# zhouxian/act3d-chained-diffuser

Measured on AMD Instinct MI355X. Metric: train samples/sec (Act3D keypose fwd+bwd+AdamW step), higher is better.
Workload: dtype fp16 / bf16 MFMA on two-part operands (x = hi + lo; fp32 accumulate) in attention; fp32-accurate linears (f32 MFMA; bf16x3 MFMA from 4096 rows); bf16 frozen backbone + FPN; 1 GPU; Act3D keypose training step, 18-PerAct-task shapes: 4 cameras 256x256, 3 ghost-point levels, 1000 ghost points (333/level), E=60, frozen synthetic CLIP-RN50-shaped backbone + trainable FPN included in the step; per_gpu_batch_keyframes=64, global_batch=64, parallelism=dp1, hipgraph=True, backbone_prefetch=True

## Files before the change

### act3d-chained-diffuser_amd/build.py

```python
import os
import shutil
import subprocess
import sys
from concurrent.futures import ThreadPoolExecutor

PKG_DIR = os.path.dirname(os.path.abspath(__file__))
CSRC = os.path.join(PKG_DIR, "csrc")
OBJ_DIR = os.path.join(CSRC, "obj")
_OUT = os.path.basename(os.environ.get("A3D_LIB_OUT", "libact3d_hip.so"))
LIB_PATH = os.path.join(PKG_DIR, _OUT)
if _OUT != "libact3d_hip.so":
    OBJ_DIR = os.path.join(CSRC, "obj_" + _OUT[len("libact3d_hip_"):-3])
INCLUDE = os.path.join(os.path.dirname(PKG_DIR), "include")
SOURCES = ["api.hip", "linear.hip", "linear_split.hip", "rope.hip", "ctx_proj.hip", "attention.hip", "attention_bwd.hip", "attention16.hip", "attention8.hip", "scene.hip", "heads.hip", "optim.hip", "diffusion.hip", "traj_rank.hip", "traj_clearance.hip", "traj_guide.hip", "vision.hip", "dropout.hip", "denoise.hip", "single_query.hip", "single_query_wave.hip", "query_stream.hip", "data.hip", "conv1x1.hip", "conv1x1_deep.hip", "bn_gram.hip", "conv3x3.hip", "fpn_sparse.hip", "stem.hip"]
FLAGS = ["--offload-arch=gfx950", "-O3", "-std=c++17", "-fPIC", "-Wno-unused-result"]
_ATTN_FLAGS = ["-fno-honor-nans", "-mno-amdgpu-ieee"]
EXTRA_FLAGS = {"attention.hip": _ATTN_FLAGS, "attention_bwd.hip": _ATTN_FLAGS, "attention16.hip": _ATTN_FLAGS,
               "attention8.hip": _ATTN_FLAGS, "traj_clearance.hip": ["-Wall", "-Wextra"],
               "traj_guide.hip": ["-Wall", "-Wextra"], "optim.hip": ["-Wall", "-Wextra"]}


ENV_FLAGS = os.environ.get("A3D_HIPCC_FLAGS", "").split()


def _hipcc():
    for cand in (shutil.which("hipcc"), "/opt/rocm/bin/hipcc"):
        if cand and os.path.exists(cand):
            return cand
    raise RuntimeError("hipcc not found: libact3d_hip.so cannot be built on this machine")


def _newer(src, dst):
    return (not os.path.exists(dst)) or os.path.getmtime(src) > os.path.getmtime(dst)


def build(force=False, verbose=False):
    hipcc = _hipcc()
    os.makedirs(OBJ_DIR, exist_ok=True)
    deps = [os.path.join(CSRC, "a3d_common.h"), os.path.join(CSRC, "attn_ring.h"), os.path.join(CSRC, "traj_points.h"),
            os.path.join(INCLUDE, "act3d_hip.h"),
            os.path.abspath(__file__)]
    srcs = [s for s in SOURCES if os.path.exists(os.path.join(CSRC, s))]
    jobs = []
    for s in srcs:
        src = os.path.join(CSRC, s)
        obj = os.path.join(OBJ_DIR, s.replace(".hip", ".o"))
        if force or _newer(src, obj) or any(_newer(d, obj) for d in deps):
            jobs.append((src, obj))

    def compile_one(job):
        src, obj = job
        cmd = [hipcc] + FLAGS + EXTRA_FLAGS.get(os.path.basename(src), []) + ENV_FLAGS + ["-c", src, "-o", obj]
        r = subprocess.run(cmd, capture_output=True, text=True)
        if r.returncode != 0:
            raise RuntimeError("hipcc failed for %s:\n%s" % (src, r.stderr[-4000:]))
        if verbose:
            print("compiled", os.path.basename(src), file=sys.stderr)
        return obj

    if jobs:
        with ThreadPoolExecutor(max_workers=min(8, len(jobs))) as ex:
            list(ex.map(compile_one, jobs))
    objs = [os.path.join(OBJ_DIR, s.replace(".hip", ".o")) for s in srcs]
    if force or jobs or not os.path.exists(LIB_PATH):
        cmd = [hipcc, "--offload-arch=gfx950", "-shared", "-fPIC", "-o", LIB_PATH] + objs
        r = subprocess.run(cmd, capture_output=True, text=True)
        if r.returncode != 0:
            raise RuntimeError("link failed:\n%s" % r.stderr[-4000:])
    return LIB_PATH


if __name__ == "__main__":
    print(build(force="--force" in sys.argv, verbose=True))
```

### act3d-chained-diffuser_amd/lib.py

```python
import ctypes as C
import os

import torch

_PKG_DIR = os.path.dirname(os.path.abspath(__file__))
LIB_PATH = os.path.join(_PKG_DIR, os.path.basename(os.environ.get("A3D_LIB", "libact3d_hip.so")))

_p = C.c_void_p
_i = C.c_int
_f = C.c_float
_d = C.c_double
_z = C.c_size_t
_u64 = C.c_ulonglong



def _struct(name, fields):
    return type(name, (C.Structure,), {"_fields_": [(f, t) for f, t in fields]})


DnHeadParams = _struct("DnHeadParams", [(n, _p) for n in ("enc_w0", "enc_b0", "enc_w1", "enc_b1", "sem", "lang_kv")] +
                       [("S_lang", _i)] + [(n, _p) for n in ("q_w", "q_b", "out_w", "out_b", "ln_g", "ln_b")])
DnCrossParams = _struct("DnCrossParams", [(n, _p) for n in ("sem", "mod", "q_w", "q_b", "freq", "Kf", "Vt")])
DnRestParams = _struct("DnRestParams", [(n, _p) for n in (
# ... 58 lines not shown
    "a3d_traj_clearance_ws_floats": (_z, [_i] * 5),
    "a3d_traj_clearance": (_i, [_p, _p, _p, _p, _i, _i, _f, _i, _i, _p, _p, _p] + [_i] * 5 + [_p]),
    "a3d_traj_guide_ws_floats": (_z, [_i] * 5),
    "a3d_traj_guide": (_i, [_p, _i, _p, _p, _p, _p, _p, _i, _i, _f, _i, _i, _f, _f, _p, _p] + [_i] * 4 + [_p]),
    "a3d_traj_errors": (_i, [_p, _p, _p, _i, _i, _i, _p]),
    "a3d_keypose_errors": (_i, [_p, _p, _p, _p, _i, _p, _i, _i, _i, _p]),
    "a3d_sym_quat_loss": (_i, [_p, _p, _i, _f, _p, _p, _i, _p]),
    "a3d_sq_fwd_ws_floats": (_z, [_i, _i, _i, _i]),
    "a3d_sq_attn_fwd": (_i, [_p, _p, _p, _i, _p, _p, _i, _p, _p, _p, _p, _p, _p, _p, _i, _i, _i, _i, _i, _p]),
    "a3d_sq_bwd_ws_floats": (_z, [_i, _i, _i, _i]),
    "a3d_sq_attn_bwd": (_i, [_p, _p, _p, _i, _p, _p, _i, _p, _p, _p, _p, _p, _p, _p, _p, _p, _i, _p, _p, _i, _p, _i, _i, _i, _i,
                             _i, _p]),
    "a3d_sq_attn_bwd_acc": (_i, [_p, _p, _p, _i, _p, _p, _i, _p, _p, _p, _p, _p, _p, _p, _p, _p, _i, _p, _p, _i, _p, _i, _i, _i, _i,
                                 _i, _i, _p]),
    "a3d_qs_pre_fwd": (_i, [_p, _p, _p, _p, _p, _f, _p, _i, _i, _i, _p]),
    "a3d_qs_pre_bwd": (_i, [_p, _i, _p, _p, _f, _p, _p, _p, _p, _p, _i, _i, _i, _p]),
    "a3d_qs_save_floats": (_z, [_i, _i]),
    "a3d_qs_post_fwd": (_i, [_p, _p, _p, _p, _p, _i, _i, _i, _p]),
    "a3d_qs_post_bwd": (_i, [_p, _p, _p, _p, _p, _p, _p, _p, _p, _i, _i, _i, _p]),
    "a3d_sq_wgrad_reduce": (_i, [_p, _i, _p, _i, _p, _i, _p]),
    "a3d_dn_head": (_i, [_p, _i, _p, _p, _i, _i, _i, _i, _p]),
    "a3d_dn_cross_ws_floats": (_z, [_i, _i, _i]),
    "a3d_dn_cross": (_i, [_p, _p, _i, _p, _p, _i, _i, _i, _i, _i, _i, _i, _p]),
    "a3d_dn_rest": (_i, [_p, _p, _i, _p, _p, _p, _i, _i, _i, _i, _i, _p]),
    "a3d_dn_tail": (_i, [_p, _p, _p, _i, _p, _p, _i, _i, _i, _i, _p]),
    "a3d_dn_tail_sched": (_i, [_p, _p, _p, _i, _p, _p, _i, _i, _i, _i, _i, _p]),
    "a3d_dn_persist_splits": (_i, [_i, _i]),
    "a3d_dn_persist_sync_ints": (_z, [_i, _i, _i, _i]),
    "a3d_dn_persist_kvx_floats": (_z, [_i, _i, _i]),
    "a3d_dn_persist_prof": (_i, [_p, _i, _i, _i, _i, _p]),
    "a3d_dn_persist_xbuf_floats": (_z, [_i, _i]),
    "a3d_dn_persist": (_i, [_p, _i, _i, _i, _p, _p, _p, _p, _p, _p, _p, _p] + [_i] * 10 + [_p]),
    "a3d_dn_persist_sched": (_i, [_p, _i, _i, _i, _p, _p, _p, _p, _p, _p, _p, _p] + [_i] * 12 + [_p]),
    "a3d_dn_persist_group_of": (_i, [_i, _i, _i, _i, _p]),
    "a3d_dn_persist_group": (_i, [_p, _i, _i, _i, _p, _p, _p, _p, _p, _p, _p, _p] + [_i] * 13 + [_p]),
    "a3d_rope_rows_f32": (_i, [_p, _i, _p, _p, _f, _p, _i, _i, _i, _i, _i, _p]),
    "a3d_dropout": (_i, [_p, _p, _z, _p, C.c_uint, _f, _p]),
    "a3d_dropout_mask": (_i, [_p, _z, _p, C.c_uint, C.c_uint, C.c_uint, _f, _p]),
    "a3d_linear_fwd_drop": (_i, [_p, _i, _p, _i, _p, _p, _i, _p, _i, _i, _i, _i, _i, _i, _p, C.c_uint, _f, _p]),
    "a3d_add_layernorm_bwd_drop": (_i, [_p] * 10 + [_i, _i, _p, C.c_uint, _f, _p]),
    "a3d_attn_fwd_dropout": (_i, [_p, _p, _p, _p, _p, _p, _p, _i, _i, _i, _i, _i, _i, _i, _p, C.c_uint, _f, _p]),
    "a3d_attn_bwd_bf16_dropout": (_i, [_p] * 15 + [_i] * 7 + [_p, C.c_uint, _f, _p]),
    "a3d_pcd_downsample": (_i, [_p, _p, _i, _i, _i, _i, _i, _p]),
    "a3d_knn_topk_ws_bytes": (_z, [_i, _i]),
    "a3d_knn_topk": (_i, [_p, _p, _p, _p, _p, _i, _i, _i, _p]),
    "a3d_traj_nn_topk": (_i, [_p, _i, _p, _p, _p, _p, _i, _i, _i, _p]),
    "a3d_build_context": (_i, [_p, _p, _p, _p, _i, _i, _i, _i, _i, _p]),
    "a3d_build_context_bwd": (_i, [_p, _p, _p, _p, _i, _i, _i, _i, _i, _i, _p]),
    "a3d_build_context_bf16": (_i, [_p, _i, _p, _p, _p, _p, _i, _i, _i, _i, _i, _p]),
    "a3d_colsum_rows_ws_floats": (_z, [_i, _i, _i]),
    "a3d_colsum_rows": (_i, [_p, _i, _i, _i, _i, _i, _p, _i, _p, _p]),
    "a3d_build_context_bwd_bf16": (_i, [_p, _p, _p, _i, _p, _i, _i, _i, _i, _i, _i, _p]),
    "a3d_mask_logits_fwd": (_i, [_p, _p, _p, _i, _i, _i, _p]),
    "a3d_mask_logits_bwd": (_i, [_p, _p, _p, _p, _p, _i, _i, _i, _i, _p]),
    "a3d_argmax_gather": (_i, [_p, _p, _p, _p, _i, _i, _p]),
    "a3d_soft_ce_loss": (_i, [_p, _p, _p, _p, _p, _p, _i, _i, _f, _f, _f, _p]),
    "a3d_elem_loss": (_i, [_p, _p, _i, _i, _f, _p, _p, _p]),
    "a3d_scale_by_scalar": (_i, [_p, _p, _p, _z, _p]),
    "a3d_quat_sigmoid_fwd": (_i, [_p, _p, _p, _i, _p]),
    "a3d_quat_sigmoid_bwd": (_i, [_p, _p, _p, _p, _i, _p]),
    "a3d_ortho6d_sigmoid_fwd": (_i, [_p, _p, _p, _i, _p]),
    "a3d_ortho6d_sigmoid_bwd": (_i, [_p, _p, _p, _p, _i, _p]),
    "a3d_select_row_fwd": (_i, [_p, _p, _p, _i, _i, _i, _p]),
    "a3d_select_row_bwd": (_i, [_p, _p, _p, _i, _i, _i, _p]),
    "a3d_sample_ghost_points": (_i, [_p, _p, _p, _f, _p, _i, _i, _i, _i, _p]),
    "a3d_rng_advance": (_i, [_p, _u64, _p]),
    "a3d_philox4x32_10_host": (None, [_p, _p, _p]),
    "a3d_sincos_host": (None, [_p, _p, _p, _z]),
    "a3d_adamw_step": (_i, [_p, _p, _p, _p, _p, _p, _p, _i, _z, _z, _f, _f, _f, _f, _f, _f, _f, _p]),
    "a3d_adamw_ema_step": (_i, [_p] * 9 + [_i, _z, _z] + [_f] * 9 + [_p]),
    "a3d_adamw_clip_step": (_i, [_p] * 11 + [_i, _z, _z] + [_f] * 10 + [_p]),
    "a3d_adamw_sched_step": (_i, [_p] * 12 + [_i, _z, _z, _i] + [_d] * 3 + [_f] * 9 + [_p]),
    "a3d_swap_f32": (_i, [_p, _p, _z, _p]),
    "a3d_dbg_mfma_bf16": (_i, [_p, _p, _p, _p]),
    "a3d_dbg_mfma_f32": (_i, [_p, _p, _p, _p]),
    "a3d_dbg_cvt_pk_bf16": (_i, [_p, _p, _i, _p]),
    "a3d_bn_nslab": (_i, [_z, _i]),
    "a3d_bn_grid_cap": (_i, [_i]),
    "a3d_conv1x1_streams": (_i, [_i, _i]),
    "a3d_conv1x1_nslab": (_i, [_z, _i, _i]),
    "a3d_conv1x1_bn_fwd": (_i, [_p, _p, _p, _p, _i, _p, _p, _z, _i, _i, _p]),
    "a3d_conv1x1_topdown_serves": (_i, [_i, _i]),
    "a3d_conv1x1_topdown_fwd": (_i, [_p, _p, _p, _i, _p, _p, _z, _i, _i, _i, _i, _p]),
    "a3d_conv1x1_bn_residual_serves": (_i, [_i, _i]),
    "a3d_conv1x1_bn_residual_fwd": (_i, [_p, _p, _p, _p, _i, _p, _p, _p, _p, _p, _i, _i, _p, _z, _i, _i, _p]),
    "a3d_bn_gram_nslab": (_i, [_z, _i]),
    "a3d_bn_gram": (_i, [_p, _p, _p, _i, _p, _p, _z, _i, _i, _p]),
    "a3d_bn_gram_stats": (_i, [_p, _p, _i, _p, _i, _i, _p, _p, _p]),
    "a3d_conv3x3_serves": (_i, [_i, _i, _i, _i]),
    "a3d_conv1x1_deep_mode": (_i, [_i]),
    "a3d_stem_conv_nslab": (_i, [_z, _i, _i]),
    "a3d_stem_conv_bn_fwd": (_i, [_p, _p, _p, _p, _p, _p, _z, _i, _i, _p]),
    "a3d_conv3x3_nslab": (_i, [_z, _i, _i, _i, _i]),
    "a3d_conv3x3_bn_fwd": (_i, [_p, _p, _p, _p, _i, _p, _p, _z, _i, _i, _i, _i, _p]),
    "a3d_bn_stats": (_i, [_p, _p, _z, _i, _i, _p]),
    "a3d_bn_finalize": (_i, [_p, _i, _z, _i, _f, _f, _p, _p, _p, _p, _p, _p, _i, _p]),
    "a3d_bn_apply": (_i, [_p, _p, _p, _p, _p, _p, _p, _z, _i, _i, _p]),
    "a3d_bn_apply_pool2": (_i, [_p, _p, _p, _p, _p, _p, _i, _i, _i, _i, _i, _p]),
    "a3d_rgb_normalize_nhwc_bf16": (_i, [_p, _p, _p, _p, _z, _i, _i, _p]),
    "a3d_upsample2_add_fwd": (_i, [_p, _p, _p, _i, _p, _i, _i, _i, _i, _p]),
    "a3d_upsample2_add_bwd_ws_floats": (_z, [_i, _i, _i, _i]),
    "a3d_upsample2_add_bwd": (_i, [_p, _p, _p, _i, _p, _i, _i, _i, _i, _p]),
    "a3d_ddpm_add_noise": (_i, [_p, _p, _p, _p, _p, _p, _i, _i, _i, _i, _p]),
    "a3d_ddpm_step": (_i, [_p, _p, _p, _p, _p, _p, _p, _p, _i, _i, _i, _i, _p]),
    "a3d_ddpm_step_sched": (_i, [_p, _p, _p, _p, _p, _p, _p, _p, _i, _i, _i, _i, _i, _p]),
    "a3d_adaln_fwd": (_i, [_p, _p, _p, _i, _i, _i, _p]),
    "a3d_adaln_bwd": (_i, [_p, _p, _p, _p, _p, _i, _i, _i, _p]),
    "a3d_sinusoidal_emb": (_i, [_p, _p, _i, _i, _p]),
    "a3d_silu_fwd": (_i, [_p, _p, _z, _p]),
    "a3d_silu_bwd": (_i, [_p, _p, _p, _z, _p]),
    "a3d_add_rows": (_i, [_p, _p, _p, _i, _i, _i, _p]),
    "a3d_add_rows_bwd": (_i, [_p, _p, _i, _i, _i, _p]),
    "a3d_resize_crop": (_i, [_p, _p, _p, _i, _i, _i, _i, _f, _f, _p]),
    "a3d_traj_update": (_i, [_p, _p, _p, _i, _i, _i, _p]),
}

ADAMW_CLIP_WS_DOUBLES = 256
LR_DECAY_KINDS = {"constant": 0, "linear": 1, "cosine": 2}

_lib = None


def load():
    global _lib
    if _lib is not None:
        return _lib
    if not os.path.exists(LIB_PATH):
        raise RuntimeError(
            "libact3d_hip.so is missing (%s). Build it with `python -c 'import __graft_entry__ as g; g.build()'` "
            "(needs hipcc); there is no CPU fallback." % LIB_PATH)
    lib = C.CDLL(LIB_PATH)
    for name, (res, args) in SIGNATURES.items():
        try:
            fn = getattr(lib, name)
        except AttributeError as e:
            raise RuntimeError("libact3d_hip.so does not export %s (stale build?)" % name) from e
        fn.restype = res
        fn.argtypes = args
    _lib = lib
    return lib


def exported_symbols():
    return list(SIGNATURES.keys())


def last_error():
    s = load().a3d_last_error_string()
    return s.decode() if s else ""


def check(rc, what=""):
    if rc != 0:
        raise RuntimeError("libact3d_hip %s failed with code %d: %s" % (what, rc, last_error()))


def ptr(t):
    if t is None:
        return None
    assert t.is_contiguous(), "libact3d_hip needs contiguous tensors"
    return t.data_ptr()


def stream():
    return torch.cuda.current_stream().cuda_stream

# ... 14 lines not shown
```

### act3d-chained-diffuser_amd/nn.py

```python
import collections
import math
import os

import torch
import torch.nn as nn
import torch.nn.functional as F

from . import ops as O


class MultiheadCustomAttention(nn.Module):

    def __init__(self, embed_dim, num_heads, dropout=0.0):
        super().__init__()
        assert embed_dim % num_heads == 0 and embed_dim // num_heads == 15, \
            "the HIP attention kernels are specialised for head_dim 15 (60/4, 120/8), as in both reference models"
        self.embed_dim, self.num_heads, self.dropout = embed_dim, num_heads, dropout
        self.in_proj_weight = nn.Parameter(torch.empty(3 * embed_dim, embed_dim))
        self.in_proj_bias = nn.Parameter(torch.zeros(3 * embed_dim))
        self.out_proj = nn.Linear(embed_dim, embed_dim)
        nn.init.xavier_uniform_(self.in_proj_weight)
        nn.init.constant_(self.out_proj.bias, 0.0)


# ... 89 lines not shown
                                    nn.Linear(4 * d_model, d_model), nn.Dropout(dropout))
        self.norm_122 = nn.LayerNorm(d_model)

    def forward(self, seq1, seq1_key_padding_mask, seq2, seq1_xyz=None, seq2_xyz=None, seq1_sem_pos=None, silu_t=None,
                drop=None, cross_cache=None):
        cached = cross_cache is not None
        if self.training and self.dropout_p > 0 and drop is None and not cached:
            raise RuntimeError("ParallelAttentionLayer in training mode with dropout=%g needs the forward pass's DropCtx "
                               "(DiffusionHead.begin_dropout())" % self.dropout_p)
        if drop is not None and (cached or not self.training or self.dropout_p <= 0):
            drop = None
        sb = self.site_base
        rope = self.rotary_pe
        q1 = seq1 if seq1_sem_pos is None else O.AddRowsFn.apply(seq1, seq1_sem_pos)
        qa = self.adaln_12(q1, silu_t) if (self.adaln_12 is not None and silu_t is not None) else q1
        if cached:
            seq1 = O.attn_block_cached(qa, seq1, seq1_xyz if rope else None, cross_cache, self.cross_12, self.norm_12, self.n_heads)
        else:
            seq1 = O.attn_block(qa, seq2, seq2, seq1, seq1_xyz if rope else None, seq2_xyz if rope else None, None,
                                self.cross_12, self.norm_12, self.n_heads, drop=drop, site=sb, sink=getattr(seq2, "_a3d_sink", None))
        if self.self_attention1:
            q1 = seq1 if seq1_sem_pos is None else O.AddRowsFn.apply(seq1, seq1_sem_pos)
            if self.adaln_1 is not None and silu_t is not None:
                qk, vv = self.adaln_1(q1, silu_t), self.adaln_1(seq1, silu_t)
            else:
                qk, vv = q1, seq1
            seq1 = O.attn_block(qk, qk, vv, seq1, seq1_xyz if rope else None, seq1_xyz if rope else None,
                                seq1_key_padding_mask, self.sa1, self.norm_1, self.n_heads, drop=drop, site=0 if cached else sb + 2)
        if self.apply_ffn:
            y = self.adaln_ff1(seq1, silu_t) if (self.adaln_ff1 is not None and silu_t is not None) else seq1
            seq1 = O.mlp(y, self.ffn_12[0], self.ffn_12[3], self.norm_122, drop=drop, site_hidden=sb + 4, site_out=sb + 5)
        return seq1


class ParallelAttention(nn.Module):
    def __init__(self, num_layers=1, **kw):
        super().__init__()
        self.layers = nn.ModuleList([ParallelAttentionLayer(**kw) for _ in range(num_layers)])

    def forward(self, seq1, seq1_key_padding_mask, seq2, cross_caches=None, **kw):
        for i, layer in enumerate(self.layers):
            seq1 = layer(seq1, seq1_key_padding_mask, seq2, cross_cache=None if cross_caches is None else cross_caches[i], **kw)
        return seq1


class _Upsample2AddFn(torch.autograd.Function):

    @staticmethod
    def forward(ctx, lat, top, bias):
        N, C, H, W = lat.shape
        y = torch.empty_like(lat)
        O.L.call("a3d_upsample2_add_fwd", lat.data_ptr(), None if top is None else top.data_ptr(),
                 None if bias is None else bias.data_ptr(), 0 if bias is None else bias.numel(), y.data_ptr(), N, H, W, C,
                 O.L.stream())
        ctx.bias = bias
        ctx.has_top = top is not None
        return y

    @staticmethod
    def backward(ctx, dy):
        dy, dtop = _top_down_backward(dy, ctx.bias, ctx.has_top and ctx.needs_input_grad[1])
        return (dy if ctx.needs_input_grad[0] else None), dtop, None


def _top_down_backward(dy, bias, want_top):
    N, C, H, W = dy.shape
    want_bias = bias is not None and bias.requires_grad
    dtop = None
    if want_top or want_bias:
        dy = dy.contiguous(memory_format=torch.channels_last)
        if want_top:
            dtop = torch.empty((N, C, H // 2, W // 2), device=dy.device, dtype=dy.dtype, memory_format=torch.channels_last)
        ws = gb = None
        if want_bias:
            ws = torch.empty((O.L.load().a3d_upsample2_add_bwd_ws_floats(N, H, W, C),), device=dy.device, dtype=torch.float32)
            gb = O.grad_buf(bias)
        O.L.call("a3d_upsample2_add_bwd", dy.data_ptr(), None if dtop is None else dtop.data_ptr(),
                 None if gb is None else gb.data_ptr(), 0 if gb is None else gb.numel(), None if ws is None else ws.data_ptr(),
                 N, H, W, C, O.L.stream())
    return dy, dtop


FUSED_FPN_LATERAL = os.environ.get("A3D_FPN_LATERAL", "1") not in ("0", "", "off")
FUSED_FPN_OUT3X3 = os.environ.get("A3D_FPN_OUT3X3", "1") not in ("0", "", "off")


class _LateralTopDownFn(torch.autograd.Function):

    @staticmethod
    def forward(ctx, x, w, bias, top):
        N, K, H, W = x.shape
        Co = w.shape[0]
        w16 = w.detach().to(torch.bfloat16).reshape(Co, K).contiguous()
        y = torch.empty((N, Co, H, W), device=x.device, dtype=torch.bfloat16, memory_format=torch.channels_last)
        O.L.call("a3d_conv1x1_topdown_fwd", x.data_ptr(), w16.data_ptr(), None if bias is None else bias.data_ptr(),
                 0 if bias is None else bias.numel(), None if top is None else top.data_ptr(), y.data_ptr(), N, H, W, K, Co, O.L.stream())
        ctx.save_for_backward(x, w16)
        ctx.bias = bias
        ctx.has_top = top is not None
        return y

    @staticmethod
    def backward(ctx, dy):
        x, w16 = ctx.saved_tensors
        dy, dtop = _top_down_backward(dy, ctx.bias, ctx.has_top and ctx.needs_input_grad[3])
        need_x, need_w = ctx.needs_input_grad[0], ctx.needs_input_grad[1]
        dx = dw = None
        if need_x or need_w:
            dy = dy.contiguous(memory_format=torch.channels_last)
            w4 = w16.view(w16.shape[0], w16.shape[1], 1, 1)
            dx, dw, _ = torch.ops.aten.convolution_backward(dy, x, w4, None, (1, 1), (0, 0), (1, 1), False, (0, 0), 1, (need_x, need_w, False))
        return dx, (None if dw is None else dw.float()), None, dtop


def _fused_lateral_ok(x, Co, last):
    cl = torch.channels_last
    return bool(FUSED_FPN_LATERAL and x.is_cuda and x.dtype == torch.bfloat16 and x.dim() == 4 and x.is_contiguous(memory_format=cl)
                and O.L.load().a3d_conv1x1_topdown_serves(x.shape[1], Co)
                and (last is None or (last.dtype == torch.bfloat16 and last.is_contiguous(memory_format=cl) and last.shape[1] == Co
                                      and x.shape[-2] == 2 * last.shape[-2] and x.shape[-1] == 2 * last.shape[-1])))


def _fused_top_down_ok(lat, last, with_bias=False):
    cl = torch.channels_last
    ok = (lat.is_cuda and lat.dtype == torch.bfloat16 and lat.shape[1] % 4 == 0 and lat.shape[-2] % 2 == 0 and lat.shape[-1] % 2 == 0
          and lat.is_contiguous(memory_format=cl))
    if last is not None:
        ok = ok and (last.dtype == torch.bfloat16 and lat.shape[-2] == 2 * last.shape[-2] and lat.shape[-1] == 2 * last.shape[-1]
                     and last.is_contiguous(memory_format=cl))
    if with_bias:
        ok = ok and 256 % (lat.shape[1] // 4) == 0
    return ok


def fpn_top_down(lat, last, bias=None):
    if _fused_top_down_ok(lat, last, bias is not None):
        return _Upsample2AddFn.apply(lat, last, bias)
    if bias is not None:
        lat = lat + F.pad(bias, (0, lat.shape[1] - bias.numel())).to(lat.dtype).view(1, -1, 1, 1)
    return lat if last is None else lat + F.interpolate(last, size=lat.shape[-2:], mode="nearest")


class _LayerConv3x3Fn(torch.autograd.Function):

    @staticmethod
    def forward(ctx, x, w, cc):
        w16 = w.to(x.dtype)
        if (FUSED_FPN_OUT3X3 and x.is_cuda and x.dtype == torch.bfloat16 and x.is_contiguous(memory_format=torch.channels_last)
                and O.L.load().a3d_conv3x3_serves(x.shape[1], w16.shape[0], x.shape[2], x.shape[3])):
            w16 = w16.contiguous(memory_format=torch.channels_last)
            y = torch.empty((x.shape[0], w16.shape[0], x.shape[2], x.shape[3]), device=x.device, dtype=torch.bfloat16,
                            memory_format=torch.channels_last)
            O.L.call("a3d_conv3x3_bn_fwd", x.data_ptr(), w16.data_ptr(), None, None, 0, y.data_ptr(), None, x.shape[0], x.shape[2], x.shape[3],
                     x.shape[1], w16.shape[0], O.L.stream())
        else:
            y = F.conv2d(x, w16, None, padding=1)
        ctx.save_for_backward(x, w16)
        ctx.cc = cc
        cc.x, cc.dw, cc.dense = x, None, False
        cc.mask, cc.ntok = None, 0
        if O.SPARSE_FPN_DGRAD and ctx.needs_input_grad[0] and O.L.load().a3d_conv3x3_tile_count(x.shape[0], x.shape[2], x.shape[3]) > 0 \
                and x.shape[2] // 8 <= 255 and x.shape[3] // 32 <= 255:
            cc.mask = torch.zeros((O.L.load().a3d_conv3x3_tile_count(x.shape[0], x.shape[2], x.shape[3]),), device=x.device, dtype=torch.uint8)
        return y

    @staticmethod
    def backward(ctx, dy):
        x, w16 = ctx.saved_tensors
        cc = ctx.cc
        sparse = cc.dw is not None and not cc.dense
        need_x, need_w = ctx.needs_input_grad[0], ctx.needs_input_grad[1]
        dx = dw = None
        N, _, H, W = x.shape
        sparse_x = (need_x and sparse and cc.mask is not None and 0 < cc.ntok <= O.SPARSE_FPN_DGRAD_MAX * N * H * W and dy.dtype == torch.bfloat16)
        if sparse_x:
            dy = dy.contiguous(memory_format=torch.channels_last)
            wt = w16.flip(2, 3).permute(1, 2, 3, 0).contiguous()
            dx = torch.empty_like(x, memory_format=torch.channels_last)
            ws = torch.empty((O.L.load().a3d_conv3x3_dgrad_tiles_ws_ints(N, H, W),), device=x.device, dtype=torch.int32)
            O.L.call("a3d_conv3x3_dgrad_tiles", dy.data_ptr(), wt.data_ptr(), cc.mask.data_ptr(), ws.data_ptr(), dx.data_ptr(), N, H, W, O.L.stream())
            need_x = False
        if need_x or (need_w and not sparse):
            dy = dy.contiguous(memory_format=torch.channels_last)
            dxl, dw, _ = torch.ops.aten.convolution_backward(dy, x, w16, None, (1, 1), (1, 1), (1, 1), False, (0, 0), 1,
                                                             (need_x, need_w and not sparse, False))
            if need_x:
                dx = dxl
        if need_w and sparse:
            dw = cc.dw.permute(2, 3, 0, 1).contiguous()
        cc.dw, cc.mask = None, None
        return dx, (None if dw is None else dw.float()), None


class FeaturePyramidNetwork(nn.Module):

    def __init__(self, in_channels_list, out_channels):
        super().__init__()
        self.inner_blocks = nn.ModuleList([nn.Sequential(nn.Conv2d(c, out_channels, 1)) for c in in_channels_list])
        self.layer_blocks = nn.ModuleList(
            [nn.Sequential(nn.Conv2d(out_channels, out_channels, 3, padding=1)) for _ in in_channels_list])
        for m in self.modules():
# ... 528 lines not shown
```

### include/act3d_hip.h

```cpp
#ifndef ACT3D_HIP_H
#define ACT3D_HIP_H
#include <stddef.h>
#include <stdint.h>
#ifdef __cplusplus
extern "C" {
#endif

int a3d_version(void);
const char* a3d_last_error_string(void);

int a3d_linear_fwd(const float* X, int ldx, const float* W, int ldw, const float* bias, float* Y, int ldy,
                   const float* mask, int ldm, int M, int N, int K, int act, int w_transposed, void* stream);
int a3d_linear_wgrad(const float* dY, int lddy, const float* X, int ldx, float* dW, int lddw, float* db, int M,
                     int N, int K, void* stream);
size_t a3d_linear_wgrad_ws_bytes(int M, int N, int K, int has_bias);
int a3d_linear_wgrad_ws(const float* dY, int lddy, const float* X, int ldx, float* dW, int lddw, float* db, int M,
                        int N, int K, float* ws, size_t ws_bytes, void* stream);
int a3d_add_layernorm_fwd(const float* A, const float* R, const float* gamma, const float* beta, float* Y,
                          float* mean, float* rstd, int M, int E, float eps, void* stream);
int a3d_add_layernorm_bwd(const float* A, const float* R, const float* gamma, const float* mean, const float* rstd,
                          const float* dY, float* dS, float* dgamma, float* dbeta, int M, int E, void* stream);

int a3d_linear_wgrad_partials(const float* dY, int lddy, const float* X, int ldx, int has_bias, int M, int N, int K,
                              float* ws, size_t ws_bytes, int* nsplit_out, void* stream);
// ... 238 lines not shown
  const void* Kf;
  const unsigned short* Vt;
} a3d_dn_cross_params;
typedef struct {
  const float *c_out_w, *c_out_b, *c_ln_g, *c_ln_b;
  const float* sem;
  const float *s_mod, *s_in_w, *s_in_b, *s_out_w, *s_out_b, *s_ln_g, *s_ln_b;
  const float* freq;
  const unsigned char* kmask;
  const float *f_mod, *f_w1, *f_b1, *f_w2, *f_b2, *f_ln_g, *f_ln_b;
  int F;
} a3d_dn_rest_params;
typedef struct {
  const float *pos_w0, *pos_b0, *pos_w1, *pos_b1, *rot_w0, *rot_b0, *rot_w1, *rot_b1;
  const float *noise, *cond_data;
  const unsigned char* cond_mask;
  const float *coef_pos, *coef_rot;
} a3d_dn_tail_params;
int a3d_dn_head(const float* traj, int D, const a3d_dn_head_params* p, float* x_out, int B, int L, int E, int H, void* stream);
size_t a3d_dn_cross_ws_floats(int B, int H, int nsplit);
int a3d_dn_cross(const float* x, const float* traj, int D, const a3d_dn_cross_params* p, float* ws, int B, int L, int E,
                 int H, int S, int Sp, int nsplit, void* stream);
int a3d_dn_rest(const float* x_in, const float* traj, int D, const float* ws, const a3d_dn_rest_params* p, float* x_out,
                int B, int L, int E, int H, int nsplit, void* stream);
int a3d_dn_tail(const float* pos_feats, const float* rot_feats, const float* traj, int D, const a3d_dn_tail_params* p,
                float* traj_out, int B, int L, int E, int t_step, void* stream);
int a3d_dn_tail_sched(const float* pos_feats, const float* rot_feats, const float* traj, int D, const a3d_dn_tail_params* p,
                      float* traj_out, int B, int L, int E, int row, int terminal, void* stream);
typedef struct {
  a3d_dn_cross_params cross;
  a3d_dn_rest_params rest;
} a3d_dn_layer_params;
int a3d_dn_persist_splits(int H, int nsplit);
size_t a3d_dn_persist_kvx_floats(int B, int L, int E);
size_t a3d_dn_persist_xbuf_floats(int B, int L);
int a3d_dn_persist_prof(const int* sync, int B, int L, int n_layers, int nsteps, long long* out256);
size_t a3d_dn_persist_sync_ints(int B, int L, int n_layers, int nsteps);
int a3d_dn_persist(const a3d_dn_layer_params* layers_dev, int n_traj, int n_pos, int n_rot, const a3d_dn_head_params* head,
                   const a3d_dn_tail_params* tail, float* traj, float* qbuf, float* part, float* kvx, float* xbuf, int* sync, int B,
                   int L, int D, int E, int H, int S, int Sp, int nsplit, int t_first, int nsteps, void* stream);
int a3d_dn_persist_sched(const a3d_dn_layer_params* layers_dev, int n_traj, int n_pos, int n_rot, const a3d_dn_head_params* head,
                         const a3d_dn_tail_params* tail, float* traj, float* qbuf, float* part, float* kvx, float* xbuf, int* sync,
                         int B, int L, int D, int E, int H, int S, int Sp, int nsplit, int row_first, int nsteps, int n_rows,
                         int last_terminal, void* stream);
int a3d_dn_persist_group_of(int B, int L, int n_cand, int traj, int* out5);
int a3d_dn_persist_group(const a3d_dn_layer_params* layers_dev, int n_traj, int n_pos, int n_rot, const a3d_dn_head_params* head,
                         const a3d_dn_tail_params* tail, float* traj, float* qbuf, float* part, float* kvx, float* xbuf, int* sync,
                         int B, int L, int D, int E, int H, int S, int Sp, int nsplit, int row_first, int nsteps, int n_rows,
                         int last_terminal, int n_cand, void* stream);
int a3d_dbg_dn_prof(long long* out18);
int a3d_rope_rows_f32(const float* Y, int ldy, const float* xyz, const float* freq, float scale, float* out, int B, int N,
                      int Npad, int E, int H, void* stream);

int a3d_bn_nslab(size_t rows, int C);
int a3d_bn_stats(const void* x, float* partial , size_t rows, int C, int nslab, void* stream);
int a3d_bn_finalize(const float* partial, int nslab, size_t rows, int C, float eps, float momentum, const float* gamma,
                    const float* beta, float* running_mean, float* running_var, float* scale, float* shift, int train,
                    void* stream);
int a3d_bn_apply(const void* x, const void* residual, const float* res_scale, const float* res_shift, const float* scale,
                 const float* shift, void* y, size_t rows, int C, int relu, void* stream);
int a3d_bn_apply_pool2(const void* x, const void* residual, const float* scale, const float* shift, void* y_full,
                       void* y_pool, int N, int H, int W, int C, int relu, void* stream);
int a3d_bn_grid_cap(int cap);
int a3d_upsample2_add_fwd(const void* lat, const void* top, const float* bias, int nbias, void* y, int N, int H, int W, int C,
                          void* stream);
size_t a3d_upsample2_add_bwd_ws_floats(int N, int H, int W, int C);
int a3d_upsample2_add_bwd(const void* dy, void* dtop, float* dbias, int nbias, float* ws, int N, int H, int W, int C,
                          void* stream);

int a3d_rgb_normalize_nhwc_bf16(const float* x, const float* mean, const float* stdv, void* y, size_t N, int H, int W,
                                void* stream);

int a3d_dbg_mfma_bf16(const void* A16x32, const void* B32x16, float* D16x16, void* stream);
int a3d_dbg_mfma_f32(const float* A16x4, const float* B4x16, float* D16x16, void* stream);
int a3d_dbg_cvt_pk_bf16(const float* in, void* out, int npairs, void* stream);

int a3d_conv1x1_streams(int K, int N);
int a3d_conv1x1_nslab(size_t M, int K, int N);
int a3d_conv1x1_bn_fwd(const void* x, const void* w, const float* in_scale, const float* in_shift, int in_relu, void* y,
                       float* partial, size_t M, int K, int N, void* stream);
int a3d_conv1x1_topdown_serves(int K, int N);
int a3d_conv1x1_topdown_fwd(const void* x, const void* w, const float* bias, int nbias, const void* top, void* y, size_t images,
                            int H, int W, int K, int N, void* stream);
int a3d_conv1x1_bn_residual_serves(int K, int N);
int a3d_conv1x1_bn_residual_fwd(const void* x, const void* w, const float* in_scale, const float* in_shift, int in_relu,
                                const float* out_scale, const float* out_shift, const void* res, const float* res_scale,
                                const float* res_shift, int relu, int round_conv, void* y, size_t M, int K, int N, void* stream);
int a3d_bn_gram_nslab(size_t M, int K);
int a3d_bn_gram(const void* x, const float* in_scale, const float* in_shift, int in_relu, float* gpart, float* spart, size_t M, int K,
                int nslab, void* stream);
int a3d_bn_gram_stats(const float* gpart, const float* spart, int nslab, const void* w, int K, int N, double* work, float* stats,
                      void* stream);
int a3d_conv1x1_deep_mode(int mode);
int a3d_stem_conv_nslab(size_t images, int H, int W);
int a3d_stem_conv_bn_fwd(const float* rgb, const float* mean, const float* stdv, const void* w, void* y, float* partial, size_t images,
                         int H, int W, void* stream);

int a3d_conv3x3_serves(int Cin, int Cout, int H, int W);
int a3d_conv3x3_nslab(size_t images, int H, int W, int Cin, int Cout);
int a3d_conv3x3_bn_fwd(const void* x, const void* w, const float* in_scale, const float* in_shift, int in_relu, void* y,
                       float* partial, size_t images, int H, int W, int Cin, int Cout, void* stream);

int a3d_resize_crop(const float* src, float* dst, const int* params, int frames, int planes, int H, int W, float scale,
                    float shift, void* stream);

#ifdef __cplusplus
}
#endif
#endif
```

Measured before the change: 3650 samples/s.

## Add fused deep-K FPN lateral 1x1 conv with upsample-add epilogue

Adds a bf16 MFMA 1x1 conv kernel for FPN lateral layers with large input channel counts (512 to 2048) and 64 output channels. It runs a persistent grid with double-buffered LDS staging and fuses bias plus the nearest-upsampled top-down map into the epilogue. Deep levels previously fell back to a library conv followed by a separate upsample-add kernel. The new path skips that extra launch and the round trip of the intermediate lateral tensor, at the cost of a hand-written kernel with tile-size heuristics. A probe script is included to compare routes and tile sizes.

```diff
diff --git a/act3d-chained-diffuser_amd/build.py b/act3d-chained-diffuser_amd/build.py
--- a/act3d-chained-diffuser_amd/build.py
+++ b/act3d-chained-diffuser_amd/build.py
@@ -12,7 +12,7 @@
 if _OUT != "libact3d_hip.so":
     OBJ_DIR = os.path.join(CSRC, "obj_" + _OUT[len("libact3d_hip_"):-3])
 INCLUDE = os.path.join(os.path.dirname(PKG_DIR), "include")
-SOURCES = ["api.hip", "linear.hip", "linear_split.hip", "rope.hip", "ctx_proj.hip", "attention.hip", "attention_bwd.hip", "attention16.hip", "attention8.hip", "scene.hip", "heads.hip", "optim.hip", "diffusion.hip", "traj_rank.hip", "traj_clearance.hip", "traj_guide.hip", "vision.hip", "dropout.hip", "denoise.hip", "single_query.hip", "single_query_wave.hip", "query_stream.hip", "data.hip", "conv1x1.hip", "conv1x1_deep.hip", "bn_gram.hip", "conv3x3.hip", "fpn_sparse.hip", "stem.hip"]
+SOURCES = ["api.hip", "linear.hip", "linear_split.hip", "rope.hip", "ctx_proj.hip", "attention.hip", "attention_bwd.hip", "attention16.hip", "attention8.hip", "scene.hip", "heads.hip", "optim.hip", "diffusion.hip", "traj_rank.hip", "traj_clearance.hip", "traj_guide.hip", "vision.hip", "dropout.hip", "denoise.hip", "single_query.hip", "single_query_wave.hip", "query_stream.hip", "data.hip", "conv1x1.hip", "conv1x1_deep.hip", "fpn_lateral.hip", "bn_gram.hip", "conv3x3.hip", "fpn_sparse.hip", "stem.hip"]
 FLAGS = ["--offload-arch=gfx950", "-O3", "-std=c++17", "-fPIC", "-Wno-unused-result"]
 _ATTN_FLAGS = ["-fno-honor-nans", "-mno-amdgpu-ieee"]
 EXTRA_FLAGS = {"attention.hip": _ATTN_FLAGS, "attention_bwd.hip": _ATTN_FLAGS, "attention16.hip": _ATTN_FLAGS,
diff --git a/act3d-chained-diffuser_amd/csrc/fpn_lateral.hip b/act3d-chained-diffuser_amd/csrc/fpn_lateral.hip
--- /dev/null
+++ b/act3d-chained-diffuser_amd/csrc/fpn_lateral.hip
@@ -0,0 +1,174 @@
+#include "a3d_common.h"
+#include "../../include/act3d_hip.h"
+
+namespace a3d {
+
+__device__ __forceinline__ int fl_woff(int row, int seg) { return row * 32 + ((seg ^ (((row >> 1) & 1) | (((row >> 4) & 1) << 1))) << 3); }
+
+typedef unsigned int u32x4 __attribute__((ext_vector_type(4)));
+
+template <int TM>
+__global__ __launch_bounds__(256, 2) void fpn_lateral_deep_kernel(const unsigned short* __restrict__ x, const unsigned short* __restrict__ w,
+                                                               const float* __restrict__ bias, int nbias,
+                                                               const unsigned short* __restrict__ top, unsigned short* __restrict__ y,
+                                                               long long M, int K, int H, int W) {
+  constexpr int BM = 64 * TM, N = 64;
+  constexpr int D = 8 / TM;
+  __shared__ __attribute__((aligned(16))) unsigned short Ws[2][64 * 32];
+  __shared__ __attribute__((aligned(16))) unsigned short Xs[2][BM * 32];
+  const int t = threadIdx.x, lane = t & 63, wave = t >> 6;
+  const int li = lane & 15, g = lane >> 4;
+  const int KS = K >> 5;
+  const long long mtiles = (M + BM - 1) / BM;
+  const long long my_tiles = blockIdx.x < mtiles ? (mtiles - blockIdx.x + gridDim.x - 1) / gridDim.x : 0;
+  const long long total = my_tiles * KS;
+  if (total == 0) return;
+  float epb[16];
+#pragma unroll
+  for (int j = 0; j < 16; ++j) {
+    const int c = g * 16 + j;
+    epb[j] = (bias && c < nbias) ? bias[c] : 0.f;
+  }
+  long long ltile = blockIdx.x, lleft = total;
+  int lks = 0;
+  auto load = [&](u32x4 (&rx)[TM], u32x4& rw) {
+    const long long m0 = ltile * BM;
+#pragma unroll
+    for (int i = 0; i < TM; ++i) {
+      const int idx = t + i * 256, row = idx >> 2, seg = idx & 3;
+      const long long m = m0 + row < M ? m0 + row : M - 1;
+      rx[i] = *reinterpret_cast<const u32x4*>(x + (size_t)m * K + lks * 32 + seg * 8);
+    }
+    rw = *reinterpret_cast<const u32x4*>(w + (size_t)(t >> 2) * K + lks * 32 + (t & 3) * 8);
+    if (lleft > 1) {
+      --lleft;
+      if (++lks == KS) { lks = 0; ltile += gridDim.x; }
+    }
+  };
+  auto stage = [&](int buf, const u32x4 (&rx)[TM], const u32x4& rw) {
+#pragma unroll
+    for (int i = 0; i < TM; ++i) {
+      const int idx = t + i * 256;
+      *reinterpret_cast<u32x4*>(&Xs[buf][plane_off(idx >> 2, idx & 3)]) = rx[i];
+    }
+    *reinterpret_cast<u32x4*>(&Ws[buf][fl_woff(t >> 2, t & 3)]) = rw;
+  };
+  u32x4 xr[D][TM], wr[D];
+#pragma unroll
+  for (int j = 0; j < D; ++j) load(xr[j], wr[j]);
+  f32x4 acc[4][TM];
+#pragma unroll
+  for (int a = 0; a < 4; ++a)
+#pragma unroll
+    for (int b = 0; b < TM; ++b) acc[a][b] = f32x4{0.f, 0.f, 0.f, 0.f};
+  long long ctile = blockIdx.x;
+  int cks = 0;
+  for (long long s0 = 0; s0 < total; s0 += D) {
+#pragma unroll
+    for (int j = 0; j < D; ++j) {
+      if (s0 + j >= total) continue;
+      const int buf = j & 1;
+      stage(buf, xr[j], wr[j]);
+      load(xr[j], wr[j]);
+      __syncthreads();
+      s16x8 xa[TM], wb[4];
+#pragma unroll
+      for (int tm = 0; tm < TM; ++tm)
+        xa[tm] = *reinterpret_cast<const s16x8*>(&Xs[buf][plane_off(wave * 16 * TM + tm * 16 + li, g)]);
+#pragma unroll
+      for (int tn = 0; tn < 4; ++tn)
+        wb[tn] = *reinterpret_cast<const s16x8*>(&Ws[buf][fl_woff((li >> 2) * 16 + tn * 4 + (li & 3), g)]);
+      const bool last = cks == KS - 1;
+      const long long m0 = ctile * BM;
+      uint4 tv[TM][2];
+      if (last && top) {
+#pragma unroll
+        for (int tm = 0; tm < TM; ++tm) {
+          const long long m = m0 + wave * 16 * TM + tm * 16 + li;
+          const unsigned int mm = (unsigned int)(m < M ? m : M - 1);
+          const unsigned int hq = mm / (unsigned int)W, w_ = mm - hq * (unsigned int)W;
+          const unsigned int n_ = hq / (unsigned int)H, h_ = hq - n_ * (unsigned int)H;
+          const size_t tr = ((size_t)n_ * (H >> 1) + (h_ >> 1)) * (W >> 1) + (w_ >> 1);
+          const uint4* src = reinterpret_cast<const uint4*>(top + tr * N + g * 16);
+          tv[tm][0] = src[0];
+          tv[tm][1] = src[1];
+        }
+      }
+#pragma unroll
+      for (int tn = 0; tn < 4; ++tn)
+#pragma unroll
+        for (int tm = 0; tm < TM; ++tm) acc[tn][tm] = mfma_bf16_16x16x32(wb[tn], xa[tm], acc[tn][tm]);
+      if (last) {
+#pragma unroll
+        for (int tm = 0; tm < TM; ++tm) {
+          const long long m = m0 + wave * 16 * TM + tm * 16 + li;
+          unsigned int pk[8];
+#pragma unroll
+          for (int tn = 0; tn < 4; ++tn) {
+#pragma unroll
+            for (int r2 = 0; r2 < 2; ++r2) {
+              float a0 = acc[tn][tm][2 * r2] + epb[4 * tn + 2 * r2];
+              float a1 = acc[tn][tm][2 * r2 + 1] + epb[4 * tn + 2 * r2 + 1];
+              if (top) {
+                const uint4 q = tv[tm][tn >> 1];
+                const unsigned int tw = (tn & 1) ? (r2 ? q.w : q.z) : (r2 ? q.y : q.x);
+                a0 += __uint_as_float(tw << 16);
+                a1 += __uint_as_float(tw & 0xFFFF0000u);
+              }
+              pk[2 * tn + r2] = pk_bf16(a0, a1);
+            }
+            acc[tn][tm] = f32x4{0.f, 0.f, 0.f, 0.f};
+          }
+          if (m < M) {
+            uint4* dst = reinterpret_cast<uint4*>(y + (size_t)m * N + g * 16);
+            dst[0] = make_uint4(pk[0], pk[1], pk[2], pk[3]);
+            dst[1] = make_uint4(pk[4], pk[5], pk[6], pk[7]);
+          }
+        }
+      }
+      if (++cks == KS) { cks = 0; ctile += gridDim.x; }
+    }
+  }
+}
+
+}
+
+using namespace a3d;
+
+static int fl_tile_mode = 0;
+extern "C" int a3d_conv1x1_lateral_deep_tile(int tm) {
+  const int prev = fl_tile_mode;
+  if (tm == 0 || tm == 1 || tm == 2 || tm == 4) fl_tile_mode = tm;
+  return prev;
+}
+static int lateral_deep_tm(size_t M) {
+  if (fl_tile_mode) return fl_tile_mode;
+  for (int tm = 4; tm > 1; tm >>= 1)
+    if ((M + 64 * tm - 1) / (64 * tm) >= 512) return tm;
+  return 1;
+}
+
+extern "C" int a3d_conv1x1_lateral_deep_serves(int K, int N) { return (N == 64 && K >= 512 && K <= 2048 && (K % 64) == 0) ? 1 : 0; }
+
+extern "C" int a3d_conv1x1_lateral_deep_fwd(const void* x, const void* w, const float* bias, int nbias, const void* top, void* y,
+                                            size_t images, int H, int W, int K, int N, void* stream) {
+  const size_t M = images * (size_t)H * (size_t)W;
+  if (!x || !w || !y || images == 0 || H <= 0 || W <= 0 || K <= 0 || N <= 0 || !a3d_conv1x1_lateral_deep_serves(K, N) || M > 0xFFFFFFFFull ||
+      (top && ((H & 1) || (W & 1))) || (bias && (nbias <= 0 || nbias > N)) ||
+      ((((uintptr_t)x | (uintptr_t)w | (uintptr_t)y | (uintptr_t)top) & 15) != 0)) {
+    set_error("a3d_conv1x1_lateral_deep_fwd: bad argument (images=%zu H=%d W=%d K=%d N=%d nbias=%d; served: K = 64 j in 512 .. 2048, N = 64, "
+              "H and W even with a top map, at most 2^32 rows, 0 < nbias <= N with a bias, 16-byte aligned operands)", images, H, W, K, N, nbias);
+    return A3D_ERR_ARG;
+  }
+  const int tm = lateral_deep_tm(M);
+  const size_t mtiles = (M + 64 * tm - 1) / (64 * tm);
+  const dim3 grid((unsigned int)std::min<size_t>(mtiles, 512));
+  hipStream_t s = (hipStream_t)stream;
+  const unsigned short *xp = (const unsigned short*)x, *wp = (const unsigned short*)w, *tp = (const unsigned short*)top;
+  unsigned short* yp = (unsigned short*)y;
+  const int nb = bias ? nbias : 0;
+  if (tm == 4) hipLaunchKernelGGL(fpn_lateral_deep_kernel<4>, grid, dim3(256), 0, s, xp, wp, bias, nb, tp, yp, (long long)M, K, H, W);
+  else if (tm == 2) hipLaunchKernelGGL(fpn_lateral_deep_kernel<2>, grid, dim3(256), 0, s, xp, wp, bias, nb, tp, yp, (long long)M, K, H, W);
+  else hipLaunchKernelGGL(fpn_lateral_deep_kernel<1>, grid, dim3(256), 0, s, xp, wp, bias, nb, tp, yp, (long long)M, K, H, W);
+  return check_launch("a3d_conv1x1_lateral_deep_fwd");
+}
diff --git a/act3d-chained-diffuser_amd/lib.py b/act3d-chained-diffuser_amd/lib.py
--- a/act3d-chained-diffuser_amd/lib.py
+++ b/act3d-chained-diffuser_amd/lib.py
@@ -164,6 +164,9 @@
     "a3d_conv1x1_bn_fwd": (_i, [_p, _p, _p, _p, _i, _p, _p, _z, _i, _i, _p]),
     "a3d_conv1x1_topdown_serves": (_i, [_i, _i]),
     "a3d_conv1x1_topdown_fwd": (_i, [_p, _p, _p, _i, _p, _p, _z, _i, _i, _i, _i, _p]),
+    "a3d_conv1x1_lateral_deep_serves": (_i, [_i, _i]),
+    "a3d_conv1x1_lateral_deep_fwd": (_i, [_p, _p, _p, _i, _p, _p, _z, _i, _i, _i, _i, _p]),
+    "a3d_conv1x1_lateral_deep_tile": (_i, [_i]),
     "a3d_conv1x1_bn_residual_serves": (_i, [_i, _i]),
     "a3d_conv1x1_bn_residual_fwd": (_i, [_p, _p, _p, _p, _i, _p, _p, _p, _p, _p, _i, _i, _p, _z, _i, _i, _p]),
     "a3d_bn_gram_nslab": (_i, [_z, _i]),
diff --git a/act3d-chained-diffuser_amd/nn.py b/act3d-chained-diffuser_amd/nn.py
--- a/act3d-chained-diffuser_amd/nn.py
+++ b/act3d-chained-diffuser_amd/nn.py
@@ -195,6 +195,7 @@
 
 
 FUSED_FPN_LATERAL = os.environ.get("A3D_FPN_LATERAL", "1") not in ("0", "", "off")
+FUSED_FPN_LATERAL_DEEP = os.environ.get("A3D_FPN_LATERAL_DEEP", "1") not in ("0", "", "off")
 FUSED_FPN_OUT3X3 = os.environ.get("A3D_FPN_OUT3X3", "1") not in ("0", "", "off")
 
 
@@ -206,7 +207,8 @@
         Co = w.shape[0]
         w16 = w.detach().to(torch.bfloat16).reshape(Co, K).contiguous()
         y = torch.empty((N, Co, H, W), device=x.device, dtype=torch.bfloat16, memory_format=torch.channels_last)
-        O.L.call("a3d_conv1x1_topdown_fwd", x.data_ptr(), w16.data_ptr(), None if bias is None else bias.data_ptr(),
+        entry = "a3d_conv1x1_topdown_fwd" if O.L.load().a3d_conv1x1_topdown_serves(K, Co) else "a3d_conv1x1_lateral_deep_fwd"
+        O.L.call(entry, x.data_ptr(), w16.data_ptr(), None if bias is None else bias.data_ptr(),
                  0 if bias is None else bias.numel(), None if top is None else top.data_ptr(), y.data_ptr(), N, H, W, K, Co, O.L.stream())
         ctx.save_for_backward(x, w16)
         ctx.bias = bias
@@ -229,7 +231,8 @@
 def _fused_lateral_ok(x, Co, last):
     cl = torch.channels_last
     return bool(FUSED_FPN_LATERAL and x.is_cuda and x.dtype == torch.bfloat16 and x.dim() == 4 and x.is_contiguous(memory_format=cl)
-                and O.L.load().a3d_conv1x1_topdown_serves(x.shape[1], Co)
+                and (O.L.load().a3d_conv1x1_topdown_serves(x.shape[1], Co)
+                     or (FUSED_FPN_LATERAL_DEEP and O.L.load().a3d_conv1x1_lateral_deep_serves(x.shape[1], Co)))
                 and (last is None or (last.dtype == torch.bfloat16 and last.is_contiguous(memory_format=cl) and last.shape[1] == Co
                                       and x.shape[-2] == 2 * last.shape[-2] and x.shape[-1] == 2 * last.shape[-1])))
 
diff --git a/include/act3d_hip.h b/include/act3d_hip.h
--- a/include/act3d_hip.h
+++ b/include/act3d_hip.h
@@ -344,6 +344,10 @@
 int a3d_conv1x1_topdown_serves(int K, int N);
 int a3d_conv1x1_topdown_fwd(const void* x, const void* w, const float* bias, int nbias, const void* top, void* y, size_t images,
                             int H, int W, int K, int N, void* stream);
+int a3d_conv1x1_lateral_deep_serves(int K, int N);
+int a3d_conv1x1_lateral_deep_fwd(const void* x, const void* w, const float* bias, int nbias, const void* top, void* y, size_t images,
+                                 int H, int W, int K, int N, void* stream);
+int a3d_conv1x1_lateral_deep_tile(int tm);
 int a3d_conv1x1_bn_residual_serves(int K, int N);
 int a3d_conv1x1_bn_residual_fwd(const void* x, const void* w, const float* in_scale, const float* in_shift, int in_relu,
                                 const float* out_scale, const float* out_shift, const void* res, const float* res_scale,
diff --git a/profiles/fpn_lateral_probe.py b/profiles/fpn_lateral_probe.py
--- /dev/null
+++ b/profiles/fpn_lateral_probe.py
@@ -0,0 +1,83 @@
+import importlib
+import json
+import os
+import sys
+
+import torch
+import torch.nn.functional as F
+
+sys.path.insert(0, os.path.dirname(os.path.dirname(os.path.abspath(__file__))))
+a3d = importlib.import_module("act3d-chained-diffuser_amd")
+L = a3d.lib
+IMAGES, N, NB, ITERS, REPS, ROT = 256, 64, 60, 8, 7, 4
+LEVELS = [("res3", 32, 512, True), ("res4", 16, 1024, True), ("res5", 8, 2048, False)]
+
+
+def timed(fn):
+    for i in range(ITERS):
+        fn(i)
+    torch.cuda.synchronize()
+    ms = []
+    for _ in range(REPS):
+        e0, e1 = torch.cuda.Event(enable_timing=True), torch.cuda.Event(enable_timing=True)
+        e0.record()
+        for i in range(ITERS):
+            fn(i)
+        e1.record()
+        torch.cuda.synchronize()
+        ms.append(e0.elapsed_time(e1) / ITERS)
+    ms.sort()
+    return {"median_us": 1e3 * ms[len(ms) // 2], "min_us": 1e3 * ms[0], "max_us": 1e3 * ms[-1]}
+
+
+def main():
+    dev = torch.device("cuda:0")
+    cl = torch.channels_last
+    lib = L.load()
+    out = {"images": IMAGES, "iters": ITERS, "reps": REPS, "levels": {}}
+    for name, S, K, with_top in LEVELS:
+        xs = [torch.randn(IMAGES, K, S, S, device=dev).to(torch.bfloat16).contiguous(memory_format=cl) for _ in range(ROT)]
+        tops = [torch.randn(IMAGES, N, S // 2, S // 2, device=dev).to(torch.bfloat16).contiguous(memory_format=cl) if with_top else None
+                for _ in range(ROT)]
+        w = torch.randn(NB, K, 1, 1, device=dev) * K ** -0.5
+        bias = torch.randn(NB, device=dev)
+        y = torch.empty((IMAGES, N, S, S), device=dev, dtype=torch.bfloat16).contiguous(memory_format=cl)
+        w16 = F.pad(w, (0, 0, 0, 0, 0, 0, 0, N - NB)).to(torch.bfloat16).reshape(N, K).contiguous()
+        nbytes = 2 * IMAGES * S * S * (K + N) + (2 * IMAGES * (S // 2) ** 2 * N if with_top else 0)
+
+        def new(i):
+            x, top = xs[i % ROT], tops[i % ROT]
+            L.call("a3d_conv1x1_lateral_deep_fwd", x.data_ptr(), w16.data_ptr(), bias.data_ptr(), NB, None if top is None else top.data_ptr(),
+                   y.data_ptr(), IMAGES, S, S, K, N, L.stream())
+
+        def new_with_cast(i):
+            x, top = xs[i % ROT], tops[i % ROT]
+            wc = F.pad(w, (0, 0, 0, 0, 0, 0, 0, N - NB)).to(torch.bfloat16).reshape(N, K).contiguous()
+            L.call("a3d_conv1x1_lateral_deep_fwd", x.data_ptr(), wc.data_ptr(), bias.data_ptr(), NB, None if top is None else top.data_ptr(),
+                   y.data_ptr(), IMAGES, S, S, K, N, L.stream())
+
+        def old(i):
+            x, top = xs[i % ROT], tops[i % ROT]
+            lat = F.conv2d(x, F.pad(w, (0, 0, 0, 0, 0, 0, 0, N - NB)).to(torch.bfloat16))
+            L.call("a3d_upsample2_add_fwd", lat.data_ptr(), None if top is None else top.data_ptr(), bias.data_ptr(), NB, y.data_ptr(),
+                   IMAGES, S, S, N, L.stream())
+
+        lv = {"K": K, "rows": IMAGES * S * S, "bytes": nbytes, "library_route": timed(old)}
+        for tile in (0, 1, 2, 4):
+            prev = lib.a3d_conv1x1_lateral_deep_tile(tile)
+            r = timed(new)
+            lib.a3d_conv1x1_lateral_deep_tile(prev)
+            r["TBps"] = nbytes / (r["median_us"] * 1e-6) / 1e12
+            lv["tile_%d" % tile] = r
+        lv["deep_entry_with_weight_cast"] = timed(new_with_cast)
+        lv["library_route"]["TBps"] = nbytes / (lv["library_route"]["median_us"] * 1e-6) / 1e12
+        out["levels"][name] = lv
+        print(name, json.dumps(lv), flush=True)
+        del xs, tops
+    path = sys.argv[1] if len(sys.argv) > 1 else os.path.join(os.path.dirname(os.path.abspath(__file__)), "fpn_lateral_probe.json")
+    with open(path, "w") as f:
+        json.dump(out, f, indent=1)
+
+
+if __name__ == "__main__":
+    main()
```

New measurement: 3625 samples/s. About the same (-0.7%).
